# wenbowen123/iros20-6d-pose-tracking

Hardware: NVIDIA H100
Metric: rgbd_pair_frames_per_sec (higher is better)
Workload: dtype bf16x3 (bf16 hi/lo split operands, 3 products/MAC, fp32 accumulate)

## Files before the change

include/se3tn.h:

```cpp
#ifndef SE3TN_H
#define SE3TN_H

#include <stddef.h>
#include <stdint.h>

#ifdef __cplusplus
extern "C" {
#endif

typedef struct se3tn_ctx se3tn_ctx;

enum {
    SE3TN_OK = 0,
    SE3TN_ERR_INVALID = -1,
    SE3TN_ERR_CUDA = -2,
    SE3TN_ERR_NOMEM = -3,
    SE3TN_ERR_STATE = -4,
    SE3TN_ERR_UNSUPPORTED = -5
};

enum {
    SE3TN_PREC_TF32 = 0,
    SE3TN_PREC_FP32 = 1,
    SE3TN_PREC_BF16X3 = 2,
// ... 102 lines not shown

int se3tn_track_render_host(se3tn_ctx* ctx, const uint8_t* frame_rgb, const uint16_t* frame_depth, int H, int W, const double* K,
                            const double* poses, const double* object_width, int render_mode, int render_H, int render_W,
                            const int32_t* weight_ids, int n, double trans_normalizer, double rot_normalizer, int precision,
                            double* poses_out, float* out_trans, float* out_rot, void* stream);


int se3tn_eval_pairs(se3tn_ctx* ctx, const uint8_t* rgbA, const uint16_t* depthA, const uint8_t* rgbB, const uint16_t* depthB,
                     const double* A_in_cam, const double* B_in_cam,
                     const int32_t* weight_ids_host, const int32_t* weight_ids_dev, int n,
                     double trans_normalizer, double rot_normalizer, int precision,
                     float* out_trans, float* out_rot, float* out_sq, double* out_labels, float* out_sums, void* stream);

int se3tn_pair_loss(se3tn_ctx* ctx, const float* trans, const float* rot, const double* trans_label, const double* rot_label, int n,
                    float* out_sums, void* stream);


int se3tn_debug_buffer(se3tn_ctx* ctx, int id, float** ptr, size_t* floats_per_image);

#define SE3TN_PROFILE_SLOTS 22
int se3tn_set_profiling(se3tn_ctx* ctx, int enable);
int se3tn_get_profile(se3tn_ctx* ctx, float* ms);

#define SE3TN_TRACE_WORDS (14 * 256 * 8)
int se3tn_get_trace(se3tn_ctx* ctx, unsigned long long* out);

int se3tn_last_step_was_graph(se3tn_ctx* ctx);
int se3tn_last_launch_count(se3tn_ctx* ctx);

#ifdef __cplusplus
}
#endif
#endif
```

iros20-6d-pose-tracking_b200/_lib.py:

```python
import ctypes as C
import os

_HERE = os.path.dirname(os.path.abspath(__file__))
LIB_PATH = os.path.join(_HERE, 'libse3tn.so')

OK, ERR_INVALID, ERR_CUDA, ERR_NOMEM, ERR_STATE, ERR_UNSUPPORTED = 0, -1, -2, -3, -4, -5
PREC_TF32, PREC_FP32, PREC_BF16X3, PREC_BF16 = 0, 1, 2, 3
RENDER_VISPY, RENDER_PYRENDER = 0, 1
WEIGHT_BLOB_FLOATS = 13528326
PROFILE_SLOTS = 22

_vp, _i, _d, _sz = C.c_void_p, C.c_int, C.c_double, C.c_size_t

SIGNATURES = {
    'se3tn_workspace_bytes': (_sz, [_i]),
    'se3tn_create': (_i, [_i, _i, _vp, C.POINTER(_vp)]),
    'se3tn_destroy': (None, [_vp]),
    'se3tn_last_error': (C.c_char_p, [_vp]),
    'se3tn_load_weights': (_i, [_vp, _i, _vp, _sz]),
    'se3tn_set_stats': (_i, [_vp, _i, _vp, _vp, _i]),
    'se3tn_preprocess': (_i, [_vp, _vp, _vp, _i, _i, _vp, _vp, _vp, _vp, _vp, _vp, _i, _i, _vp, _vp, _vp, _vp, _vp]),
    'se3tn_normalize': (_i, [_vp, _vp, _vp, _vp, _vp, _vp, _vp, _i, _i, _vp, _vp, _vp]),
    'se3tn_compute_bbox': (_i, [_vp, _vp, _vp, _vp, _vp, _vp, _i, _vp]),
    'se3tn_crop_bbox': (_i, [_vp, _vp, _vp, _i, _i, _vp, _i, _i, _i, _vp, _vp, _vp]),
    'se3tn_forward': (_i, [_vp, _i, _vp, _vp, _i, _vp, _vp, _vp, _i, _vp]),
    'se3tn_forward_preprocessed': (_i, [_vp, _i, _i, _i, _vp, _vp, _vp, _i, _vp]),
    'se3tn_pose_update': (_i, [_vp, _vp, _vp, _vp, _d, _d, _vp, _i, _vp]),
    'se3tn_so3_log': (_i, [_vp, _vp, _vp, _d, _d, _vp, _vp, _i, _vp]),
    'se3tn_track_batch': (_i, [_vp, _vp, _vp, _i, _i, _vp, _vp, _vp, _vp, _vp, _vp, _vp, _i, _d, _d, _i, _vp, _vp, _vp, _vp]),
    'se3tn_add_adi': (_i, [_vp, _vp, _i, _vp, _vp, _i, _vp, _vp, _vp]),
    'se3tn_vocap': (_i, [_vp, _vp, _i, C.POINTER(_d), _vp]),
    'se3tn_allgather_poses': (_i, [_vp, _vp, _vp, _vp, _i, _vp]),
    'se3tn_upload_frame_window': (_i, [_vp, _vp, _vp, _i, _i, _i, _i, _i, _i, _vp, _vp, _vp]),
# ... 53 lines not shown
```

iros20-6d-pose-tracking_b200/csrc/conv_common.h:

```cpp
#pragma once
#include <cstdint>
#include <cuda.h>
#include <cuda_runtime.h>

namespace se3tn {

constexpr int kMaxTaps = 9;
constexpr int kBlockM = 128;
constexpr int kChunkBytes = 128;

enum Act : int { ACT_NONE = 0, ACT_RELU = 1, ACT_SELU = 2 };
enum { KIND_S1 = 0, KIND_S2 = 1, KIND_STEM = 2 };

struct Tap {
    int16_t dy, dx;
};

struct ConvGeom {
    int Hin, Win, in_cstride, in_coff;
    int Ho, Wo, stride;
    int cin;
    int cout;
    int groups;
    int num_taps;
// ... 49 lines not shown
    int n_layers;
    int total_units;
    int img_first, n_img;
    int max_batch;
    unsigned* sched;
    const int* img_wid;
    const CUtensorMap* gbmaps;
    const float* const* gbias;
    unsigned long long* trace;
    int ksplit;
    float* partial;
    unsigned* slice_cnt;
};

struct ResidentParams {
    LayerDesc L;
    int img_first, n_img;
    int m_tiles;
    int step_x, step_y, off_x, off_y;
    const int* img_wid;
    const CUtensorMap* gbmaps;
    const float* const* gbias;
    unsigned long long* trace;
};

cudaError_t launch_conv_resident(const ResidentParams& p, int kind, int prec, int num_sms, bool pdl, cudaStream_t stream);
cudaError_t launch_conv_trunk(const TrunkParams& p, int prec, int num_sms, bool pdl, cudaStream_t stream);
constexpr int kSplitMaxImages = 4, kSplitK = 4, kSplitMaxUnits = kSplitMaxImages * 8 * kTrunkMaxLayers;
inline size_t trunk_sched_words(int max_batch) { return 1 + static_cast<size_t>(kTrunkMaxLayers) * max_batch + static_cast<size_t>(kSplitMaxUnits) * 4; }
inline size_t trunk_partial_floats() { return static_cast<size_t>(kSplitMaxUnits) * kSplitK * 128 * 128; }

cudaError_t launch_conv_direct(const ConvGeom& g, const ConvPtrs& p, cudaStream_t stream);

}
```

iros20-6d-pose-tracking_b200/csrc/conv_wgmma.cu:

```cuda
#include "conv_common.h"
#include "ptx.cuh"
#include "storage.cuh"
#include <algorithm>

namespace se3tn {
namespace {

constexpr int kThreads2 = 384;
constexpr int kPoolPitch = 68;
constexpr int kPoolStageBytes = 121 * kPoolPitch * 4;
constexpr int kPoolStageAlloc = (kPoolStageBytes + 1023) & ~1023;
constexpr int kAUnit3 = 19 * 1024;
constexpr int kAUnitStem = 21 * 1024;
constexpr int kWgRowBytes = 64 * kChunkBytes;

template <int KIND> struct KTab;
template <> struct KTab<KIND_S1> {
    static constexpr int NU = 3;
    __host__ __device__ static constexpr int ntaps(int) { return 3; }
    __host__ __device__ static constexpr int wtap(int u, int k) { return k * 3 + u; }
    __host__ __device__ static constexpr int amap(int) { return 0; }
    __host__ __device__ static constexpr int c1(int u) { return u - 1; }
    __host__ __device__ static constexpr int c2(int) { return -1; }
    __host__ __device__ static constexpr int rows(int) { return 11 * 13; }
// ... 13 lines not shown
    __host__ __device__ static constexpr int wtap(int u, int k) { return 2 * k + u; }
    __host__ __device__ static constexpr int amap(int u) { return u; }
    __host__ __device__ static constexpr int c1(int) { return 0; }
    __host__ __device__ static constexpr int c2(int) { return 0; }
    __host__ __device__ static constexpr int rows(int u) { return u == 0 ? 11 * 14 : 11 * 13; }
};
constexpr int kRowShift = 11;

__device__ __forceinline__ float selu_fast(float x) {
    constexpr float kAlpha = 1.6732632423543772f, kScale = 1.0507009873554805f;
    return x > 0.f ? kScale * x : (kScale * kAlpha) * (__expf(x) - 1.f);
}
__device__ __forceinline__ float act_apply(float x, int act) {
    return act == ACT_RELU ? fmaxf(x, 0.f) : (act == ACT_SELU ? selu_fast(x) : x);
}

__device__ __forceinline__ unsigned long long gtimer() { unsigned long long t; asm volatile("mov.u64 %0, %%globaltimer;" : "=l"(t)); return t; }
__device__ __forceinline__ void trace_stamp(unsigned long long* tr, int slot) { if (tr) tr[blockIdx.x * 8 + slot] = gtimer(); }
__device__ __forceinline__ void trace_exit(unsigned long long* tr) {
    if (!tr) return;
    unsigned smid; asm volatile("mov.u32 %0, %%smid;" : "=r"(smid));
    tr[blockIdx.x * 8 + 7] = (gtimer() & ~0xffull) | (smid & 0xff);
}

using ptx::desc_lo;
using ptx::mk_desc;

__device__ __forceinline__ float (&acc_lo32(float (&d)[64]))[32] { return *reinterpret_cast<float (*)[32]>(&d[0]); }

struct Consumer {
    int ct, cg, cw, ew, lane, R, m;
    __device__ __forceinline__ Consumer() {
        ct = static_cast<int>(threadIdx.x) - 128; cg = ct >> 7; ew = ct >> 5; cw = ew & 3; lane = ct & 31; R = lane >> 2; m = lane & 3;
    }
    __device__ __forceinline__ bool leader() const { return (ct & 127) == 0; }
    __device__ __forceinline__ int row(int h) const { return 64 * cg + 16 * cw + R + 8 * h; }
};

template <int KIND, int PREC> struct RCfg {
    static constexpr bool POOL = (KIND == KIND_STEM);
    static constexpr int BN = 64;
    static constexpr int kStack = ((POOL ? stem_input_prec(PREC) : PREC) == SE3TN_PREC_BF16X3) ? 2 : 1;
    static constexpr int kBTile = BN * kStack * kChunkBytes;
    static constexpr int kAUnit = POOL ? kAUnitStem : kAUnit3;
    static constexpr int kAStages = POOL ? (PREC == SE3TN_PREC_TF32 ? 4 : 3) : (PREC == SE3TN_PREC_BF16 ? 6 : 4);
    static constexpr int kPoolBufs = POOL ? (PREC == SE3TN_PREC_TF32 ? 2 : 1) : 0;
    static constexpr int kAcc = BN * kStack / 2;
    static constexpr int kMaxWTiles = POOL ? 7 : ((PREC == SE3TN_PREC_TF32) ? 18 : 9);
    static constexpr int kSmem = kAStages * kAUnit + kMaxWTiles * kBTile + kPoolBufs * kPoolStageAlloc + 1024 + 512;
    static_assert(kSmem <= 232448, "shared memory budget");
};

template <int KIND, int PREC>
__device__ __forceinline__ void resident_mma_unit(float (&acc)[RCfg<KIND, PREC>::kAcc], uint32_t a_unit_lo, const uint8_t* sB,
                                                  int u, int ch, int tiles_per_tap, uint32_t& fresh)
{
    using C = RCfg<KIND, PREC>;
    using KT = KTab<KIND>;
#pragma unroll
    for (int k = 0; k < 4; ++k) {
// ... 2 lines not shown
        uint32_t b_lo;
        if (C::kStack == 2) b_lo = desc_lo(sB + KT::wtap(u, k) * C::kBTile) + ch * 4;
        else                b_lo = desc_lo(sB + (KT::wtap(u, k) * tiles_per_tap + ch) * C::kBTile);
        if constexpr (PREC == SE3TN_PREC_TF32) {
#pragma unroll
            for (int kk = 0; kk < 4; ++kk) ptx::wgmma_tf32_n64(acc, mk_desc(a_lo + 2 * kk), mk_desc(b_lo + 2 * kk), fresh | (kk ? 1u : 0u));
        } else if constexpr (C::POOL) {
#pragma unroll
            for (int kk = 0; kk < 4; ++kk) ptx::wgmma_bf16_n128(acc, mk_desc(a_lo + 2 * kk), mk_desc(b_lo + 2 * kk), fresh | (kk ? 1u : 0u));
        } else if constexpr (C::kStack == 2) {
#pragma unroll
            for (int sl = 0; sl < 2; ++sl) {
                ptx::wgmma_bf16_n128(acc, mk_desc(a_lo + 2 * sl), mk_desc(b_lo + 2 * sl), fresh | (sl ? 1u : 0u));
                ptx::wgmma_bf16_n64(acc_lo32(acc), mk_desc(a_lo + 4 + 2 * sl), mk_desc(b_lo + 2 * sl), 1u);
            }
        } else {
#pragma unroll
            for (int kk = 0; kk < 4; ++kk) ptx::wgmma_bf16_n64(acc, mk_desc(a_lo + 2 * kk), mk_desc(b_lo + 2 * kk), fresh | (kk ? 1u : 0u));
        }
        fresh = 1u;
    }
}

template <int KIND, int PREC>
__global__ void __launch_bounds__(kThreads2, 1)
conv_resident_kernel(const __grid_constant__ ResidentParams p)
{
    using C = RCfg<KIND, PREC>;
    using KT = KTab<KIND>;
    constexpr bool POOL = C::POOL;
    extern __shared__ uint8_t smem_raw[];
    uint8_t* smem = reinterpret_cast<uint8_t*>((reinterpret_cast<uintptr_t>(smem_raw) + 1023) & ~uintptr_t(1023));
    const LayerDesc& L = p.L;
    const int chunks = L.chunks;
    const int tiles_per_tap = (C::kStack == 2) ? 1 : chunks;
    uint8_t* sA = smem;
    uint8_t* sB = sA + C::kAStages * C::kAUnit;
    uint8_t* sP = sB + C::kMaxWTiles * C::kBTile;
    uint64_t* bars = reinterpret_cast<uint64_t*>(sP + C::kPoolBufs * kPoolStageAlloc);
    uint64_t* a_full = bars;
    uint64_t* a_empty = a_full + C::kAStages;
    uint64_t* b_full = a_empty + C::kAStages;
    uint64_t* b_empty = b_full + KT::NU;

    ptx::grid_dep_launch();
    if (threadIdx.x == 0) trace_stamp(p.trace, 0);
    const int warp = threadIdx.x >> 5;
    const int lane = threadIdx.x & 31;
    const int tiles_img = L.tiles_x * L.tiles_y;
    const int w_begin = static_cast<int>(static_cast<long long>(blockIdx.x) * p.m_tiles / gridDim.x);
    const int w_end = static_cast<int>(static_cast<long long>(blockIdx.x + 1) * p.m_tiles / gridDim.x);
    auto img_of = [&](int tile) -> int { return p.img_first + tile / tiles_img; };
    auto wid_of = [&](int tile) -> int { return p.img_wid ? p.img_wid[img_of(tile)] : -1; };

    if (threadIdx.x == 0) {
        for (int s = 0; s < C::kAStages; ++s) { ptx::mbar_init(&a_full[s], 1); ptx::mbar_init(&a_empty[s], 2); }
        for (int u = 0; u < KT::NU; ++u) ptx::mbar_init(&b_full[u], 1);
        ptx::mbar_init(&b_empty[0], 2);
        ptx::fence_barrier_init();
        ptx::fence_proxy_async();
    }
    __syncthreads();
    if (threadIdx.x == 0) trace_stamp(p.trace, 1);

    if (warp == 0) {
        if (lane == 0) {
            ptx::grid_dep_wait();
            int stage = 0; uint32_t phase = 0;
            for (int tile = w_begin; tile < w_end; ++tile) {
                const int n0 = img_of(tile), r = tile % tiles_img;
                const int ty = r / L.tiles_x, tx = r - ty * L.tiles_x;
                const int ox = tx * p.step_x + p.off_x, oy = ty * p.step_y + p.off_y;
                for (int ch = 0; ch < chunks; ++ch) {
#pragma unroll
                    for (int u = 0; u < KT::NU; ++u) {
                        ptx::mbar_wait(&a_empty[stage], phase ^ 1);
                        ptx::mbar_arrive_expect_tx(&a_full[stage], static_cast<uint32_t>(KT::rows(u)) * kChunkBytes);
                        ptx::tma_load_4d(sA + stage * C::kAUnit, &L.amap[KT::amap(u)], &a_full[stage],
                                         ch * 32, ox + KT::c1(u), oy + KT::c2(u), n0);
                        if (++stage == C::kAStages) { stage = 0; phase ^= 1; }
                    }
                }
            }
        }
    } else if (warp == 1) {
        if (lane == 0) {
            int cur = -2; uint32_t gen = 0;
            for (int tile = w_begin; tile < w_end; ++tile) {
                const int wid = wid_of(tile);
                if (wid == cur) continue;
                if (gen) ptx::mbar_wait(&b_empty[0], (gen - 1) & 1);
                const CUtensorMap* bm = wid < 0 ? &L.bmap : p.gbmaps + wid * kLayersPerSet + L.li;
#pragma unroll
                for (int u = 0; u < KT::NU; ++u) {
                    ptx::mbar_arrive_expect_tx(&b_full[u], static_cast<uint32_t>(KT::ntaps(u) * tiles_per_tap) * C::kBTile);
#pragma unroll
                    for (int k = 0; k < KT::ntaps(u); ++k)
                        for (int c = 0; c < tiles_per_tap; ++c) {
                            const int wt = KT::wtap(u, k) * tiles_per_tap + c;
                            ptx::tma_load_2d(sB + wt * C::kBTile, bm, &b_full[u], wt * 32, 0);
                        }
                }
                cur = wid; ++gen;
            }
        }
    } else if (warp >= 4) {
        ptx::grid_dep_wait();
        const Consumer cs;
        const bool stamp = threadIdx.x == 128;
        int astage = 0; uint32_t aphase = 0;
        int w_cur = -2; uint32_t w_gen = 0;
        int it = 0;
        for (int tile = w_begin; tile < w_end; ++tile, ++it) {
            const int wid = wid_of(tile);
            const bool new_w = (wid != w_cur);
            const int n0 = img_of(tile), r = tile % tiles_img;
            const int ty = r / L.tiles_x, tx = r - ty * L.tiles_x;

            using S = Storage<PREC>;
            size_t rpix[2]; bool rvalid[2]; Raw<PREC, 8> rres[2][2];
            if constexpr (!POOL) {
#pragma unroll
                for (int h = 0; h < 2; ++h) {
                    const int rw = cs.row(h);
                    const int py = rw / 11, px = rw - py * 11;
                    const int y = ty * 11 + py, x = tx * 11 + px;
                    rvalid[h] = (rw < 121) && (y < L.Ho) && (x < L.Wo);
                    rpix[h] = (static_cast<size_t>(n0) * L.Ho + y) * L.Wo + x;
#pragma unroll
                    for (int b = 0; b < 2; ++b) {
                        rres[h][b] = Raw<PREC, 8>{};
                        if (L.res && rvalid[h]) {
                            const uint8_t* rp = L.res + S::addr(rpix[h], L.res_c, 32 * b + 8 * cs.m);
#pragma unroll
                            for (int q = 0; q < rres[h][b].kPieces; ++q) rres[h][b].set(q, __ldg(rres[h][b].at(rp, q)));
                        }
                    }
                }
            }

            float acc[C::kAcc];
#pragma unroll
            for (int i = 0; i < C::kAcc; ++i) acc[i] = 0.f;
            uint32_t fresh = 0;
            int pend = -1;
            for (int ch = 0; ch < chunks; ++ch) {
#pragma unroll
                for (int u = 0; u < KT::NU; ++u) {
                    if (new_w && ch == 0) {
                        ptx::mbar_wait(&b_full[u], w_gen & 1);
                        if (it == 0 && u == 0 && stamp) trace_stamp(p.trace, 2);
                    }
                    ptx::mbar_wait(&a_full[astage], aphase);
                    if (it == 0 && ch == 0 && u == 0 && stamp) trace_stamp(p.trace, 3);
                    ptx::wgmma_fence();
                    resident_mma_unit<KIND, PREC>(acc, desc_lo(sA + astage * C::kAUnit + cs.cg * kWgRowBytes), sB, u, ch, tiles_per_tap, fresh);
                    ptx::wgmma_commit();
                    ptx::wgmma_wait<1>();
                    if (pend >= 0 && cs.leader()) ptx::mbar_arrive(&a_empty[pend]);
                    pend = astage;
                    if (++astage == C::kAStages) { astage = 0; aphase ^= 1; }
                }
            }
            ptx::wgmma_wait<0>();
            ptx::wgmma_reg_fence(acc);
            if (cs.leader()) {
                ptx::mbar_arrive(&a_empty[pend]);
                if (tile + 1 < w_end && wid_of(tile + 1) != wid) ptx::mbar_arrive(&b_empty[0]);
            }
            if (new_w) { w_cur = wid; ++w_gen; }
            if (it == 0 && stamp) trace_stamp(p.trace, 5);

            if constexpr (!POOL) {
#pragma unroll
                for (int b = 0; b < 2; ++b) {
                    const int ch0 = 32 * b + 8 * cs.m;
                    const float* bias_base = (p.img_wid ? p.gbias[p.img_wid[n0] * kLayersPerSet + L.li] : L.bias) + ch0;
                    const float4 bA = __ldg(reinterpret_cast<const float4*>(bias_base)), bB = __ldg(reinterpret_cast<const float4*>(bias_base + 4));
                    const float bias8[8] = {bA.x, bA.y, bA.z, bA.w, bB.x, bB.y, bB.z, bB.w};
#pragma unroll
                    for (int h = 0; h < 2; ++h) {
                        if (!rvalid[h]) continue;
                        float v[8];
#pragma unroll
                        for (int jj = 0; jj < 4; ++jj)
#pragma unroll
                            for (int e = 0; e < 2; ++e) {
                                const int ri = 16 * b + 4 * jj + 2 * h + e;
                                float a = acc[ri];
                                if constexpr (C::kStack == 2) a += acc[32 + ri];
                                v[2 * jj + e] = a + bias8[2 * jj + e];
                            }
                        if (L.res) {
                            float r[8];
                            S::decode(rres[h][b], r);
#pragma unroll
                            for (int e = 0; e < 8; ++e) v[e] += r[e];
                        }
#pragma unroll
                        for (int e = 0; e < 8; ++e) v[e] = act_apply(v[e], L.act);
                        S::encode(v).store(L.out + S::addr(rpix[h], L.out_c, L.out_coff + ch0));
                    }
                }
            } else {
                float* stage = reinterpret_cast<float*>(sP + (C::kPoolBufs == 2 ? (it & 1) : 0) * kPoolStageAlloc);
#pragma unroll
                for (int h = 0; h < 2; ++h) {
                    const int rw = cs.row(h);
                    if (rw >= 121) continue;
                    const int cy_l = rw / 11, cx_l = rw - cy_l * 11;
                    const int cy = ty * p.step_y + p.off_y + cy_l, cx = tx * p.step_x + p.off_x + cx_l;
                    const bool cvalid = cy >= 0 && cy < 88 && cx >= 0 && cx < 88;
                    float* srow = stage + rw * kPoolPitch + 2 * cs.m;
                    const float ninf = -3.0e38f;
#pragma unroll
                    for (int j = 0; j < 8; ++j) {
                        float a0 = acc[4 * j + 2 * h], a1 = acc[4 * j + 2 * h + 1];
                        if constexpr (C::kStack == 2) { a0 += acc[32 + 4 * j + 2 * h]; a1 += acc[32 + 4 * j + 2 * h + 1]; }
                        *reinterpret_cast<float2*>(srow + 8 * j) = cvalid ? make_float2(a0, a1) : make_float2(ninf, ninf);
                    }
                }
                asm volatile("bar.sync 1, 256;" ::: "memory");

                const float* bias = p.img_wid ? p.gbias[p.img_wid[n0] * kLayersPerSet + L.li] : L.bias;
                for (int v = cs.ct; v < 400; v += 256) {
                    const int pp = v >> 4, c4 = (v & 15) * 4;
                    const int ppy = pp / 5, ppx = pp - ppy * 5;
                    const int oy = ty * 5 + ppy, ox = tx * 5 + ppx;
                    if (oy >= L.Ho || ox >= L.Wo) continue;
                    float4 mx = make_float4(-3.0e38f, -3.0e38f, -3.0e38f, -3.0e38f);
#pragma unroll
                    for (int dy = 0; dy < 3; ++dy)
#pragma unroll
                        for (int dx = 0; dx < 3; ++dx) {
                            const float4 s4 = *reinterpret_cast<const float4*>(stage + ((2 * ppy + dy) * 11 + 2 * ppx + dx) * kPoolPitch + c4);
                            mx.x = fmaxf(mx.x, s4.x); mx.y = fmaxf(mx.y, s4.y); mx.z = fmaxf(mx.z, s4.z); mx.w = fmaxf(mx.w, s4.w);
                        }
                    const float4 b4 = __ldg(reinterpret_cast<const float4*>(bias + c4));
                    const float v4[4] = {selu_fast(mx.x + b4.x), selu_fast(mx.y + b4.y), selu_fast(mx.z + b4.z), selu_fast(mx.w + b4.w)};
                    S::encode(v4).store(L.out + S::addr((static_cast<size_t>(n0) * L.Ho + oy) * L.Wo + ox, L.out_c, L.out_coff + c4));
                }
                if (C::kPoolBufs == 1) asm volatile("bar.sync 1, 256;" ::: "memory");
            }
        }
        if (stamp) { trace_stamp(p.trace, 4); trace_stamp(p.trace, 6); }
    }

    __syncthreads();
    if (threadIdx.x == 0) trace_exit(p.trace);
}

template <int PREC> struct TCfg {
    static constexpr int BN = 128;
    static constexpr int kAcc = BN / 2;
    static constexpr int kAStages = 3;
    static constexpr int kBStages = 6;
    static constexpr int kBTile = BN * kChunkBytes;
    static constexpr int kEpiPitch = 36;
    static constexpr int kEpiWarpBytes = 16 * kEpiPitch * 4 + 128;
    static constexpr int kEpiBytes = 8 * kEpiWarpBytes;
    static constexpr int kSched = 4;
    static constexpr int kSmem = kAStages * kAUnit3 + kBStages * kBTile + ((kEpiBytes + 1023) & ~1023) + 1024 + 512;
    static_assert(kSmem <= 232448, "shared memory budget");
};
constexpr int kProducerRegs = 40;
constexpr int kConsumerRegs = 232;
constexpr int kTurnBar = 1;
constexpr int kTaps3 = 9;

__device__ __forceinline__ void ring_skip(int& stage, uint32_t& phase, int n, int stages) {
    stage += n;
    phase ^= static_cast<uint32_t>(stage / stages) & 1u;
    stage %= stages;
}

struct UnitCoord { int l, img, tx, ty, n_tile, grp, c0, c1, piece, gidx; };
__device__ __forceinline__ void unit_stamp(const TrunkParams& p, int u, int k) {
    if (p.trace && u < 2048) p.trace[256 * 8 + u * 5 + k] = k == 4 ? (gtimer() & ~0xffull) | (blockIdx.x & 0xff) : gtimer();
}

__device__ __forceinline__ int unit_layer(const TrunkParams& p, int u) {
    int l = 0;
#pragma unroll
    for (int i = 1; i < kTrunkMaxLayers; ++i) if (i < p.n_layers && u >= p.layer[i].unit_base) l = i;
    return l;
}

__device__ __forceinline__ UnitCoord decode_unit(const TrunkParams& p, int u) {
    UnitCoord c;
    c.l = unit_layer(p, u);
    const LayerDesc& L = p.layer[c.l];
    int local = u - L.unit_base;
    c.piece = 0; c.c0 = 0; c.c1 = L.chunks;
    if (p.ksplit > 1) {
        c.piece = local % p.ksplit; local /= p.ksplit;
        c.c0 = c.piece * L.chunks / p.ksplit; c.c1 = (c.piece + 1) * L.chunks / p.ksplit;
    }
// ... 395 lines not shown
    __syncthreads();
    if (threadIdx.x == 0) trace_exit(p.trace);
}

template <typename K>
cudaError_t set_smem(K kernel, size_t smem, size_t* cache) {
    int dev = 0;
    if (cudaGetDevice(&dev) != cudaSuccess || dev < 0 || dev >= 64) dev = 0;
    if (smem > cache[dev]) {
        cudaError_t e = cudaFuncSetAttribute(kernel, cudaFuncAttributeMaxDynamicSharedMemorySize, static_cast<int>(smem));
        if (e != cudaSuccess) return e;
        cache[dev] = smem;
    }
    return cudaSuccess;
}

template <int KIND, int PREC>
cudaError_t launch_resident_t(const ResidentParams& p, int num_sms, bool pdl, cudaStream_t stream) {
    using C = RCfg<KIND, PREC>;
    const int tiles_per_tap = (C::kStack == 2) ? 1 : p.L.chunks;
    if ((KIND == KIND_STEM ? 7 : 9) * tiles_per_tap > C::kMaxWTiles) return cudaErrorInvalidValue;
    if (C::kStack == 2 && KIND == KIND_S1 && p.L.chunks != 2) return cudaErrorInvalidValue;
    if (p.L.cout != 64 || p.L.groups != 1 || p.L.n_tiles != 1 || p.m_tiles <= 0) return cudaErrorInvalidValue;
    static size_t attr[64] = {};
    cudaError_t e = set_smem(conv_resident_kernel<KIND, PREC>, C::kSmem, attr);
    if (e != cudaSuccess) return e;
    cudaLaunchConfig_t cfg = {};
    cfg.gridDim = dim3(std::min(p.m_tiles, num_sms)); cfg.blockDim = dim3(kThreads2); cfg.dynamicSmemBytes = C::kSmem; cfg.stream = stream;
    cudaLaunchAttribute at[1];
    at[0].id = cudaLaunchAttributeProgrammaticStreamSerialization; at[0].val.programmaticStreamSerializationAllowed = 1;
    cfg.attrs = at; cfg.numAttrs = pdl ? 1 : 0;
    return cudaLaunchKernelEx(&cfg, conv_resident_kernel<KIND, PREC>, p);
}

template <int PREC>
cudaError_t launch_trunk_t(const TrunkParams& p, int num_sms, bool pdl, cudaStream_t stream) {
    using C = TCfg<PREC>;
    if (p.n_layers < 1 || p.n_layers > kTrunkMaxLayers || p.total_units <= 0 || !p.sched) return cudaErrorInvalidValue;
    if (p.ksplit < 1 || (p.ksplit > 1 && (!p.partial || !p.slice_cnt || p.ksplit > kSplitK))) return cudaErrorInvalidValue;
    for (int l = 0; l < p.n_layers; ++l) {
        const LayerDesc& L = p.layer[l];
        if ((L.kind != KIND_S1 && L.kind != KIND_S2) || L.cout % C::BN || L.n_tiles != L.cout / C::BN) return cudaErrorInvalidValue;
        if (L.pool_part && (L.tiles_x != 1 || L.tiles_y != 1)) return cudaErrorInvalidValue;
        if (L.dep_layer >= l) return cudaErrorInvalidValue;
        if (L.chunks % p.ksplit) return cudaErrorInvalidValue;
    }
    static size_t attr[64] = {};
    cudaError_t e = set_smem(conv_trunk_kernel<PREC>, C::kSmem, attr);
    if (e != cudaSuccess) return e;
    cudaLaunchConfig_t cfg = {};
    cfg.gridDim = dim3(std::min(p.total_units, num_sms)); cfg.blockDim = dim3(kThreads2); cfg.dynamicSmemBytes = C::kSmem; cfg.stream = stream;
    cudaLaunchAttribute at[1];
    at[0].id = cudaLaunchAttributeProgrammaticStreamSerialization; at[0].val.programmaticStreamSerializationAllowed = 1;
    cfg.attrs = at; cfg.numAttrs = pdl ? 1 : 0;
    return cudaLaunchKernelEx(&cfg, conv_trunk_kernel<PREC>, p);
// ... 32 lines not shown
```

iros20-6d-pose-tracking_b200/csrc/se3tn.cu:

```cuda
#include "../../include/se3tn.h"
#include "conv_common.h"
#include "aux_kernels.h"
#include "metrics.h"
#include "render.h"
#include <dlfcn.h>
#include "depth_fill.h"
#include "storage.cuh"

#include <algorithm>
#include <cmath>
#include <cstdio>
#include <cstdlib>
#include <cstring>
#include <map>
#include <memory>
#include <string>
#include <type_traits>
#include <vector>

using namespace se3tn;

namespace {

enum Buf { B_X0A, B_X0B, B_Y1A, B_Y1B, B_P1A, B_P1B, B_T1, B_T2, B_U, B_CAT, B_F1, B_T4, B_F2, B_H1, B_H2, B_H3, B_COUNT };
// ... 450 lines not shown
            p.w = w.blob.get() + w.w_off[li]; p.bias = w.blob.get() + w.b_off[li];
            { ProfScope ps(c, li, s); CU_TRY(c, launch_conv_direct(g, p, s)); }
            ++c->launches;
            if (li == 0) { ProfScope ps(c, 14, s); CU_TRY(c, launch_maxpool(bufp(B_Y1A), bufp(B_P1A), n, 88, 88, 64, s)); ++c->launches; }
            if (li == 1) { ProfScope ps(c, 15, s); CU_TRY(c, launch_maxpool(bufp(B_Y1B), bufp(B_P1B), n, 88, 88, 64, s)); ++c->launches; }
        }
        { ProfScope ps(c, 16, s); CU_TRY(c, launch_head(bufp(B_H3), fcw, fcw + 6 * 512, out_trans, out_rot, n, 121, s)); }
        ++c->launches;
        if (out_feature) { CU_TRY(c, launch_nhwc_to_nchw(bufp(B_F2), out_feature, n, 22 * 22, 256, precision, s)); ++c->launches; }
        return SE3TN_OK;
    }
    const CUtensorMap* gbmaps = img_wid ? c->d_bmaps[precision].get() : nullptr;
    const float* const* gbias = img_wid ? c->d_bias.get() : nullptr;
    if (c->sched_dirty) { CU_TRY(c, cudaMemsetAsync(c->sched.get(), 0, trunk_sched_words(c->max_batch) * sizeof(unsigned), s)); c->sched_dirty = false; }
    for (int li = 0; li < kFirstTrunkLayer; ++li) {
        ResidentParams rp;
        fill_layer_desc(c, w, li, precision, rp.L);
        rp.img_first = first; rp.n_img = n;
        rp.m_tiles = n * rp.L.tiles_x * rp.L.tiles_y;
        if (kLayers[li].kind == K_STEM) { rp.step_x = rp.step_y = 10; rp.off_x = rp.off_y = -1; }
        else { rp.step_x = rp.step_y = 11; rp.off_x = rp.off_y = 0; }
        rp.img_wid = img_wid; rp.gbmaps = gbmaps; rp.gbias = gbias;
        rp.trace = c->trace ? c->trace.get() + static_cast<size_t>(li) * 256 * 8 : nullptr;
        { ProfScope ps(c, li, s); CU_TRY(c, launch_conv_resident(rp, rp.L.kind, precision, c->num_sms, c->pdl != 0, s)); }
        ++c->launches;
    }
    {
        TrunkParams tp;
        memset(&tp, 0, sizeof tp);
        int ksplit = (n <= kSplitMaxImages) ? kSplitK : 1;
        for (int l = 0; l < 14 - kFirstTrunkLayer; ++l) {
            fill_layer_desc(c, w, kFirstTrunkLayer + l, precision, tp.layer[l]);
            while (tp.layer[l].chunks % ksplit) ksplit /= 2;
        }
        int base = 0, base0 = 0;
        for (int l = 0; l < 14 - kFirstTrunkLayer; ++l) {
            LayerDesc& d = tp.layer[l];
            d.unit_base = base; base += n * d.units_per_image * ksplit;
            d.base_unit0 = base0; base0 += n * d.units_per_image;
            if (l > 0) { d.dep_layer = l - 1; d.dep_target = 4u * static_cast<unsigned>(ksplit) * static_cast<unsigned>(tp.layer[l - 1].units_per_image); }
        }
        if (ksplit > 1 && base0 > kSplitMaxUnits) return fail(c, SE3TN_ERR_STATE, "split-K scratch too small");
        tp.ksplit = ksplit; tp.partial = c->partial.get();
        tp.slice_cnt = c->sched.get() + 1 + static_cast<size_t>(kTrunkMaxLayers) * c->max_batch;
        tp.layer[5].pool_part = c->pool_part.get();
        tp.n_layers = 6; tp.total_units = base;
// ... 888 lines not shown
```

iros20-6d-pose-tracking_b200/engine.py:

```python
import ctypes as C
import math
import numpy as np
import torch

from . import _lib
from .weights import pack_state_dict

PREC = {'tf32': _lib.PREC_TF32, 'fp32': _lib.PREC_FP32, 'bf16x3': _lib.PREC_BF16X3, 'bf16': _lib.PREC_BF16}
IMAGE_SIZE = 176


def _ptr(t):
    return C.c_void_p(t.data_ptr()) if t is not None else C.c_void_p(0)


def _stream(device):
    return C.c_void_p(torch.cuda.current_stream(device).cuda_stream)


class Engine:
    def __init__(self, max_batch=64, device=None):
        if not torch.cuda.is_available():
            raise RuntimeError('se3tn Engine needs a CUDA device (sm_90a); there is no CPU fallback')
        self.lib = _lib.load()
# ... 346 lines not shown
        if not (math.isfinite(max_depth) and max_depth > 0):
            raise ValueError('max_depth must be finite and > 0')
        return (1, max_depth, int(bool(fill_depth.get('extrapolate', False))), 1 if blur_type == 'gaussian' else 0)

    def _set_depth_fill(self, spec):
        _lib.check(self.lib.se3tn_set_depth_fill(self._ctx, int(spec[0]), float(spec[1]), int(spec[2]), int(spec[3])), self._ctx)

    def debug_buffer(self, buf_id, n):
        p = C.c_void_p(); fpi = C.c_size_t()
        _lib.check(self.lib.se3tn_debug_buffer(self._ctx, buf_id, C.byref(p), C.byref(fpi)), self._ctx)
        offb = p.value - self._workspace.data_ptr()
        nbytes = n * fpi.value * 4
        return self._workspace[offb:offb + nbytes].view(torch.float32).view(n, fpi.value)

    def set_profiling(self, enable=True):
        _lib.check(self.lib.se3tn_set_profiling(self._ctx, int(bool(enable))), self._ctx)

    def get_profile(self):
        ms = (C.c_float * _lib.PROFILE_SLOTS)()
        _lib.check(self.lib.se3tn_get_profile(self._ctx, ms), self._ctx)
        return np.array(ms[:], dtype=np.float64)

    def get_trace(self):
        out = np.zeros((14, 256, 8), dtype=np.uint64)
        _lib.check(self.lib.se3tn_get_trace(self._ctx, out.ctypes.data_as(C.c_void_p)), self._ctx)
        return out

    def last_launch_count(self):
        return self.lib.se3tn_last_launch_count(self._ctx)

    def last_step_was_graph(self):
        return bool(self.lib.se3tn_last_step_was_graph(self._ctx))

    def _check_img(self, t):
        if not (t.is_cuda and t.dtype == torch.float32 and t.is_contiguous() and t.dim() == 4 and
                tuple(t.shape[1:]) == (4, IMAGE_SIZE, IMAGE_SIZE)):
            raise ValueError('expected a contiguous float32 CUDA tensor of shape (n,4,176,176), got %s %s' % (t.dtype, tuple(t.shape)))

    def _check_dev(self, name, t, dtype, shape):
        if not (isinstance(t, torch.Tensor) and t.is_cuda and t.device == self.device and t.dtype == dtype and t.is_contiguous()
                and tuple(t.shape) == tuple(shape)):
            raise ValueError('%s must be a contiguous %s CUDA tensor of shape %s on %s' % (name, dtype, tuple(shape), self.device))

    def _check_frame(self, rgb, depth, rgbA, depthA, poses, ow, n):
        ok = (rgb.is_cuda and rgb.dtype == torch.uint8 and rgb.is_contiguous() and rgb.dim() == 3 and rgb.shape[2] == 3 and
              depth.is_cuda and depth.dtype == torch.uint16 and depth.is_contiguous() and depth.shape == rgb.shape[:2] and
              (rgbA is None or (rgbA.is_cuda and rgbA.dtype == torch.uint8 and rgbA.is_contiguous() and tuple(rgbA.shape) == (n, IMAGE_SIZE, IMAGE_SIZE, 3))) and
# ... 33 lines not shown
```

Measured before the change: 27570.

## Ping-pong consumer warpgroups across tiles in resident conv kernel

When a layer has more tiles than SMs, the resident conv kernel now uses a ping-pong schedule. Each consumer warpgroup owns alternate tiles and computes both 64-row halves, and named barriers hand the MMA turn back and forth. This lets one warpgroup's epilogue (bias, residual, activation, pooling) overlap the other's MMAs. Producer and consumer registers are rebalanced with setmaxnreg, and per-tile trace stamps are added for profiling. The trade-offs are higher register pressure from doubled accumulators and extra barrier synchronisation.

```diff
diff --git a/include/se3tn.h b/include/se3tn.h
--- a/include/se3tn.h
+++ b/include/se3tn.h
@@ -148,7 +148,8 @@
 int se3tn_set_profiling(se3tn_ctx* ctx, int enable);
 int se3tn_get_profile(se3tn_ctx* ctx, float* ms);
 
-#define SE3TN_TRACE_WORDS (14 * 256 * 8)
+#define SE3TN_TRACE_TILES 5184
+#define SE3TN_TRACE_WORDS (14 * 256 * 8 + 8 * SE3TN_TRACE_TILES * 4)
 int se3tn_get_trace(se3tn_ctx* ctx, unsigned long long* out);
 
 int se3tn_last_step_was_graph(se3tn_ctx* ctx);
diff --git a/iros20-6d-pose-tracking_b200/_lib.py b/iros20-6d-pose-tracking_b200/_lib.py
--- a/iros20-6d-pose-tracking_b200/_lib.py
+++ b/iros20-6d-pose-tracking_b200/_lib.py
@@ -9,6 +9,7 @@
 RENDER_VISPY, RENDER_PYRENDER = 0, 1
 WEIGHT_BLOB_FLOATS = 13528326
 PROFILE_SLOTS = 22
+TRACE_TILES = 5184
 
 _vp, _i, _d, _sz = C.c_void_p, C.c_int, C.c_double, C.c_size_t
 
diff --git a/iros20-6d-pose-tracking_b200/csrc/conv_common.h b/iros20-6d-pose-tracking_b200/csrc/conv_common.h
--- a/iros20-6d-pose-tracking_b200/csrc/conv_common.h
+++ b/iros20-6d-pose-tracking_b200/csrc/conv_common.h
@@ -95,6 +95,7 @@
     const CUtensorMap* gbmaps;
     const float* const* gbias;
     unsigned long long* trace;
+    unsigned long long* tile_trace;
 };
 
 cudaError_t launch_conv_resident(const ResidentParams& p, int kind, int prec, int num_sms, bool pdl, cudaStream_t stream);
diff --git a/iros20-6d-pose-tracking_b200/csrc/conv_wgmma.cu b/iros20-6d-pose-tracking_b200/csrc/conv_wgmma.cu
--- a/iros20-6d-pose-tracking_b200/csrc/conv_wgmma.cu
+++ b/iros20-6d-pose-tracking_b200/csrc/conv_wgmma.cu
@@ -59,6 +59,9 @@
     unsigned smid; asm volatile("mov.u32 %0, %%smid;" : "=r"(smid));
     tr[blockIdx.x * 8 + 7] = (gtimer() & ~0xffull) | (smid & 0xff);
 }
+__device__ __forceinline__ void tile_stamp(unsigned long long* tt, int tile, int k) {
+    if (tt && tile < SE3TN_TRACE_TILES) tt[tile * 4 + k] = k == 3 ? (gtimer() & ~0xffull) | (blockIdx.x & 0xff) : gtimer();
+}
 
 using ptx::desc_lo;
 using ptx::mk_desc;
@@ -71,8 +74,20 @@
         ct = static_cast<int>(threadIdx.x) - 128; cg = ct >> 7; ew = ct >> 5; cw = ew & 3; lane = ct & 31; R = lane >> 2; m = lane & 3;
     }
     __device__ __forceinline__ bool leader() const { return (ct & 127) == 0; }
-    __device__ __forceinline__ int row(int h) const { return 64 * cg + 16 * cw + R + 8 * h; }
+    __device__ __forceinline__ int row(int half, int h) const { return 64 * half + 16 * cw + R + 8 * h; }
 };
+
+constexpr int kProducerRegs = 40;
+constexpr int kConsumerRegs = 232;
+constexpr int kTurnBar = 1;
+constexpr int kStageBar = 3;
+constexpr int kEpiBar = 5;
+
+__device__ __forceinline__ void ring_skip(int& stage, uint32_t& phase, int n, int stages) {
+    stage += n;
+    phase ^= static_cast<uint32_t>(stage / stages) & 1u;
+    stage %= stages;
+}
 
 template <int KIND, int PREC> struct RCfg {
     static constexpr bool POOL = (KIND == KIND_STEM);
@@ -121,13 +136,15 @@
     }
 }
 
-template <int KIND, int PREC>
+template <int KIND, int PREC, bool PP>
 __global__ void __launch_bounds__(kThreads2, 1)
 conv_resident_kernel(const __grid_constant__ ResidentParams p)
 {
     using C = RCfg<KIND, PREC>;
     using KT = KTab<KIND>;
     constexpr bool POOL = C::POOL;
+    constexpr int NH = PP ? 2 : 1;
+    constexpr bool kShareStage = PP && C::kPoolBufs == 1;
     extern __shared__ uint8_t smem_raw[];
     uint8_t* smem = reinterpret_cast<uint8_t*>((reinterpret_cast<uintptr_t>(smem_raw) + 1023) & ~uintptr_t(1023));
     const LayerDesc& L = p.L;
@@ -153,7 +170,7 @@
     auto wid_of = [&](int tile) -> int { return p.img_wid ? p.img_wid[img_of(tile)] : -1; };
 
     if (threadIdx.x == 0) {
-        for (int s = 0; s < C::kAStages; ++s) { ptx::mbar_init(&a_full[s], 1); ptx::mbar_init(&a_empty[s], 2); }
+        for (int s = 0; s < C::kAStages; ++s) { ptx::mbar_init(&a_full[s], 1); ptx::mbar_init(&a_empty[s], PP ? 1 : 2); }
         for (int u = 0; u < KT::NU; ++u) ptx::mbar_init(&b_full[u], 1);
         ptx::mbar_init(&b_empty[0], 2);
         ptx::fence_barrier_init();
@@ -162,85 +179,117 @@
     __syncthreads();
     if (threadIdx.x == 0) trace_stamp(p.trace, 1);
 
-    if (warp == 0) {
-        if (lane == 0) {
-            ptx::grid_dep_wait();
-            int stage = 0; uint32_t phase = 0;
-            for (int tile = w_begin; tile < w_end; ++tile) {
-                const int n0 = img_of(tile), r = tile % tiles_img;
-                const int ty = r / L.tiles_x, tx = r - ty * L.tiles_x;
-                const int ox = tx * p.step_x + p.off_x, oy = ty * p.step_y + p.off_y;
-                for (int ch = 0; ch < chunks; ++ch) {
+    if (warp < 4) {
+        ptx::setmaxnreg_dec<kProducerRegs>();
+        if (warp == 0) {
+            if (lane == 0) {
+                ptx::grid_dep_wait();
+                int stage = 0; uint32_t phase = 0;
+                for (int tile = w_begin; tile < w_end; ++tile) {
+                    const int n0 = img_of(tile), r = tile % tiles_img;
+                    const int ty = r / L.tiles_x, tx = r - ty * L.tiles_x;
+                    const int ox = tx * p.step_x + p.off_x, oy = ty * p.step_y + p.off_y;
+                    for (int ch = 0; ch < chunks; ++ch) {
+#pragma unroll
+                        for (int u = 0; u < KT::NU; ++u) {
+                            ptx::mbar_wait(&a_empty[stage], phase ^ 1);
+                            ptx::mbar_arrive_expect_tx(&a_full[stage], static_cast<uint32_t>(KT::rows(u)) * kChunkBytes);
+                            ptx::tma_load_4d(sA + stage * C::kAUnit, &L.amap[KT::amap(u)], &a_full[stage],
+                                             ch * 32, ox + KT::c1(u), oy + KT::c2(u), n0);
+                            if (++stage == C::kAStages) { stage = 0; phase ^= 1; }
+                        }
+                    }
+                }
+            }
+        } else if (warp == 1) {
+            if (lane == 0) {
+                int cur = -2; uint32_t gen = 0;
+                for (int tile = w_begin; tile < w_end; ++tile) {
+                    const int wid = wid_of(tile);
+                    if (wid == cur) continue;
+                    if (gen) ptx::mbar_wait(&b_empty[0], (gen - 1) & 1);
+                    const CUtensorMap* bm = wid < 0 ? &L.bmap : p.gbmaps + wid * kLayersPerSet + L.li;
 #pragma unroll
                     for (int u = 0; u < KT::NU; ++u) {
-                        ptx::mbar_wait(&a_empty[stage], phase ^ 1);
-                        ptx::mbar_arrive_expect_tx(&a_full[stage], static_cast<uint32_t>(KT::rows(u)) * kChunkBytes);
-                        ptx::tma_load_4d(sA + stage * C::kAUnit, &L.amap[KT::amap(u)], &a_full[stage],
-                                         ch * 32, ox + KT::c1(u), oy + KT::c2(u), n0);
-                        if (++stage == C::kAStages) { stage = 0; phase ^= 1; }
-                    }
-                }
-            }
-        }
-    } else if (warp == 1) {
-        if (lane == 0) {
-            int cur = -2; uint32_t gen = 0;
-            for (int tile = w_begin; tile < w_end; ++tile) {
-                const int wid = wid_of(tile);
-                if (wid == cur) continue;
-                if (gen) ptx::mbar_wait(&b_empty[0], (gen - 1) & 1);
-                const CUtensorMap* bm = wid < 0 ? &L.bmap : p.gbmaps + wid * kLayersPerSet + L.li;
-#pragma unroll
-                for (int u = 0; u < KT::NU; ++u) {
-                    ptx::mbar_arrive_expect_tx(&b_full[u], static_cast<uint32_t>(KT::ntaps(u) * tiles_per_tap) * C::kBTile);
-#pragma unroll
-                    for (int k = 0; k < KT::ntaps(u); ++k)
-                        for (int c = 0; c < tiles_per_tap; ++c) {
-                            const int wt = KT::wtap(u, k) * tiles_per_tap + c;
-                            ptx::tma_load_2d(sB + wt * C::kBTile, bm, &b_full[u], wt * 32, 0);
-                        }
-                }
-                cur = wid; ++gen;
-            }
-        }
-    } else if (warp >= 4) {
+                        ptx::mbar_arrive_expect_tx(&b_full[u], static_cast<uint32_t>(KT::ntaps(u) * tiles_per_tap) * C::kBTile);
+#pragma unroll
+                        for (int k = 0; k < KT::ntaps(u); ++k)
+                            for (int c = 0; c < tiles_per_tap; ++c) {
+                                const int wt = KT::wtap(u, k) * tiles_per_tap + c;
+                                ptx::tma_load_2d(sB + wt * C::kBTile, bm, &b_full[u], wt * 32, 0);
+                            }
+                    }
+                    cur = wid; ++gen;
+                }
+            }
+        }
+    } else {
+        ptx::setmaxnreg_inc<kConsumerRegs>();
         ptx::grid_dep_wait();
+        using S = Storage<PREC>;
         const Consumer cs;
         const bool stamp = threadIdx.x == 128;
+        const bool tstamp = cs.leader() && (PP || cs.cg == 0);
+        constexpr int kEpiThreads = PP ? 128 : 256;
+        const int et = PP ? (cs.ct & 127) : cs.ct;
+        auto half_of = [&](int hf) { return PP ? hf : cs.cg; };
         int astage = 0; uint32_t aphase = 0;
         int w_cur = -2; uint32_t w_gen = 0;
+        if constexpr (PP) {
+            if (cs.cg == 1) { ptx::bar_arrive(kTurnBar, 256); if constexpr (kShareStage) ptx::bar_arrive(kStageBar, 256); }
+        }
         int it = 0;
         for (int tile = w_begin; tile < w_end; ++tile, ++it) {
             const int wid = wid_of(tile);
             const bool new_w = (wid != w_cur);
+            const bool w_last = tile + 1 < w_end && wid_of(tile + 1) != wid;
+            if (PP && (it & 1) != cs.cg) {
+                ring_skip(astage, aphase, chunks * KT::NU, C::kAStages);
+                if (new_w) {
+#pragma unroll
+                    for (int u = 0; u < KT::NU; ++u) ptx::mbar_wait(&b_full[u], w_gen & 1);
+                    w_cur = wid; ++w_gen;
+                }
+                if (w_last && cs.leader()) ptx::mbar_arrive(&b_empty[0]);
+                continue;
+            }
             const int n0 = img_of(tile), r = tile % tiles_img;
             const int ty = r / L.tiles_x, tx = r - ty * L.tiles_x;
 
-            using S = Storage<PREC>;
-            size_t rpix[2]; bool rvalid[2]; Raw<PREC, 8> rres[2][2];
-            if constexpr (!POOL) {
+            constexpr int kPreRes = (PP && C::kStack == 2) ? 1 : NH;
+            size_t rpix[NH][2]; bool rvalid[NH][2]; Raw<PREC, 8> rres[NH][2][2];
+            auto load_res = [&](int hf) {
 #pragma unroll
                 for (int h = 0; h < 2; ++h) {
-                    const int rw = cs.row(h);
+                    const int rw = cs.row(half_of(hf), h);
                     const int py = rw / 11, px = rw - py * 11;
                     const int y = ty * 11 + py, x = tx * 11 + px;
-                    rvalid[h] = (rw < 121) && (y < L.Ho) && (x < L.Wo);
-                    rpix[h] = (static_cast<size_t>(n0) * L.Ho + y) * L.Wo + x;
+                    rvalid[hf][h] = (rw < 121) && (y < L.Ho) && (x < L.Wo);
+                    rpix[hf][h] = (static_cast<size_t>(n0) * L.Ho + y) * L.Wo + x;
 #pragma unroll
                     for (int b = 0; b < 2; ++b) {
-                        rres[h][b] = Raw<PREC, 8>{};
-                        if (L.res && rvalid[h]) {
-                            const uint8_t* rp = L.res + S::addr(rpix[h], L.res_c, 32 * b + 8 * cs.m);
-#pragma unroll
-                            for (int q = 0; q < rres[h][b].kPieces; ++q) rres[h][b].set(q, __ldg(rres[h][b].at(rp, q)));
+                        rres[hf][h][b] = Raw<PREC, 8>{};
+                        if (L.res && rvalid[hf][h]) {
+                            const uint8_t* rp = L.res + S::addr(rpix[hf][h], L.res_c, 32 * b + 8 * cs.m);
+#pragma unroll
+                            for (int q = 0; q < Raw<PREC, 8>::kPieces; ++q) rres[hf][h][b].set(q, __ldg(Raw<PREC, 8>::at(rp, q)));
                         }
                     }
                 }
-            }
-
-            float acc[C::kAcc];
-#pragma unroll
-            for (int i = 0; i < C::kAcc; ++i) acc[i] = 0.f;
+            };
+            if constexpr (!POOL) {
+#pragma unroll
+                for (int hf = 0; hf < kPreRes; ++hf) load_res(hf);
+            }
+            float4 pb4 = make_float4(0.f, 0.f, 0.f, 0.f);
+            if constexpr (POOL) pb4 = __ldg(reinterpret_cast<const float4*>((p.img_wid ? p.gbias[p.img_wid[n0] * kLayersPerSet + L.li] : L.bias) + (et & 15) * 4));
+
+            float acc[NH][C::kAcc];
+#pragma unroll
+            for (int hf = 0; hf < NH; ++hf)
+#pragma unroll
+                for (int i = 0; i < C::kAcc; ++i) acc[hf][i] = 0.f;
+            if constexpr (PP) ptx::bar_sync(kTurnBar + cs.cg, 256);
             uint32_t fresh = 0;
             int pend = -1;
             for (int ch = 0; ch < chunks; ++ch) {
@@ -251,9 +300,18 @@
                         if (it == 0 && u == 0 && stamp) trace_stamp(p.trace, 2);
                     }
                     ptx::mbar_wait(&a_full[astage], aphase);
-                    if (it == 0 && ch == 0 && u == 0 && stamp) trace_stamp(p.trace, 3);
+                    if (ch == 0 && u == 0) {
+                        if (it == 0 && stamp) trace_stamp(p.trace, 3);
+                        if (tstamp) tile_stamp(p.tile_trace, tile, 0);
+                    }
                     ptx::wgmma_fence();
-                    resident_mma_unit<KIND, PREC>(acc, desc_lo(sA + astage * C::kAUnit + cs.cg * kWgRowBytes), sB, u, ch, tiles_per_tap, fresh);
+                    const uint32_t a_unit_lo = desc_lo(sA + astage * C::kAUnit);
+#pragma unroll
+                    for (int hf = 0; hf < NH; ++hf) {
+                        uint32_t f = fresh;
+                        resident_mma_unit<KIND, PREC>(acc[hf], a_unit_lo + half_of(hf) * (kWgRowBytes >> 4), sB, u, ch, tiles_per_tap, f);
+                    }
+                    fresh = 1u;
                     ptx::wgmma_commit();
                     ptx::wgmma_wait<1>();
                     if (pend >= 0 && cs.leader()) ptx::mbar_arrive(&a_empty[pend]);
@@ -261,68 +319,79 @@
                     if (++astage == C::kAStages) { astage = 0; aphase ^= 1; }
                 }
             }
+            if constexpr (PP) ptx::bar_arrive(kTurnBar + (cs.cg ^ 1), 256);
             ptx::wgmma_wait<0>();
-            ptx::wgmma_reg_fence(acc);
+#pragma unroll
+            for (int hf = 0; hf < NH; ++hf) ptx::wgmma_reg_fence(acc[hf]);
+            if (tstamp) tile_stamp(p.tile_trace, tile, 1);
             if (cs.leader()) {
                 ptx::mbar_arrive(&a_empty[pend]);
-                if (tile + 1 < w_end && wid_of(tile + 1) != wid) ptx::mbar_arrive(&b_empty[0]);
+                if (w_last) ptx::mbar_arrive(&b_empty[0]);
             }
             if (new_w) { w_cur = wid; ++w_gen; }
             if (it == 0 && stamp) trace_stamp(p.trace, 5);
+            if (tstamp) tile_stamp(p.tile_trace, tile, 2);
 
             if constexpr (!POOL) {
 #pragma unroll
-                for (int b = 0; b < 2; ++b) {
-                    const int ch0 = 32 * b + 8 * cs.m;
-                    const float* bias_base = (p.img_wid ? p.gbias[p.img_wid[n0] * kLayersPerSet + L.li] : L.bias) + ch0;
-                    const float4 bA = __ldg(reinterpret_cast<const float4*>(bias_base)), bB = __ldg(reinterpret_cast<const float4*>(bias_base + 4));
-                    const float bias8[8] = {bA.x, bA.y, bA.z, bA.w, bB.x, bB.y, bB.z, bB.w};
-#pragma unroll
-                    for (int h = 0; h < 2; ++h) {
-                        if (!rvalid[h]) continue;
-                        float v[8];
-#pragma unroll
-                        for (int jj = 0; jj < 4; ++jj)
-#pragma unroll
-                            for (int e = 0; e < 2; ++e) {
-                                const int ri = 16 * b + 4 * jj + 2 * h + e;
-                                float a = acc[ri];
-                                if constexpr (C::kStack == 2) a += acc[32 + ri];
-                                v[2 * jj + e] = a + bias8[2 * jj + e];
+                for (int hf = 0; hf < NH; ++hf) {
+                    if (hf >= kPreRes) load_res(hf);
+#pragma unroll
+                    for (int b = 0; b < 2; ++b) {
+                        const int ch0 = 32 * b + 8 * cs.m;
+                        const float* bias_base = (p.img_wid ? p.gbias[p.img_wid[n0] * kLayersPerSet + L.li] : L.bias) + ch0;
+                        const float4 bA = __ldg(reinterpret_cast<const float4*>(bias_base)), bB = __ldg(reinterpret_cast<const float4*>(bias_base + 4));
+                        const float bias8[8] = {bA.x, bA.y, bA.z, bA.w, bB.x, bB.y, bB.z, bB.w};
+#pragma unroll
+                        for (int h = 0; h < 2; ++h) {
+                            if (!rvalid[hf][h]) continue;
+                            float v[8];
+#pragma unroll
+                            for (int jj = 0; jj < 4; ++jj)
+#pragma unroll
+                                for (int e = 0; e < 2; ++e) {
+                                    const int ri = 16 * b + 4 * jj + 2 * h + e;
+                                    float a = acc[hf][ri];
+                                    if constexpr (C::kStack == 2) a += acc[hf][32 + ri];
+                                    v[2 * jj + e] = a + bias8[2 * jj + e];
+                                }
+                            if (L.res) {
+                                float r[8];
+                                S::decode(rres[hf][h][b], r);
+#pragma unroll
+                                for (int e = 0; e < 8; ++e) v[e] += r[e];
                             }
-                        if (L.res) {
-                            float r[8];
-                            S::decode(rres[h][b], r);
-#pragma unroll
-                            for (int e = 0; e < 8; ++e) v[e] += r[e];
+#pragma unroll
+                            for (int e = 0; e < 8; ++e) v[e] = act_apply(v[e], L.act);
+                            S::encode(v).store(L.out + S::addr(rpix[hf][h], L.out_c, L.out_coff + ch0));
                         }
-#pragma unroll
-                        for (int e = 0; e < 8; ++e) v[e] = act_apply(v[e], L.act);
-                        S::encode(v).store(L.out + S::addr(rpix[h], L.out_c, L.out_coff + ch0));
                     }
                 }
             } else {
                 float* stage = reinterpret_cast<float*>(sP + (C::kPoolBufs == 2 ? (it & 1) : 0) * kPoolStageAlloc);
-#pragma unroll
-                for (int h = 0; h < 2; ++h) {
-                    const int rw = cs.row(h);
-                    if (rw >= 121) continue;
-                    const int cy_l = rw / 11, cx_l = rw - cy_l * 11;
-                    const int cy = ty * p.step_y + p.off_y + cy_l, cx = tx * p.step_x + p.off_x + cx_l;
-                    const bool cvalid = cy >= 0 && cy < 88 && cx >= 0 && cx < 88;
-                    float* srow = stage + rw * kPoolPitch + 2 * cs.m;
-                    const float ninf = -3.0e38f;
-#pragma unroll
-                    for (int j = 0; j < 8; ++j) {
-                        float a0 = acc[4 * j + 2 * h], a1 = acc[4 * j + 2 * h + 1];
-                        if constexpr (C::kStack == 2) { a0 += acc[32 + 4 * j + 2 * h]; a1 += acc[32 + 4 * j + 2 * h + 1]; }
-                        *reinterpret_cast<float2*>(srow + 8 * j) = cvalid ? make_float2(a0, a1) : make_float2(ninf, ninf);
-                    }
-                }
-                asm volatile("bar.sync 1, 256;" ::: "memory");
-
-                const float* bias = p.img_wid ? p.gbias[p.img_wid[n0] * kLayersPerSet + L.li] : L.bias;
-                for (int v = cs.ct; v < 400; v += 256) {
+                if constexpr (kShareStage) ptx::bar_sync(kStageBar + cs.cg, 256);
+                else if constexpr (PP) ptx::bar_sync(kEpiBar + cs.cg, 128);
+#pragma unroll
+                for (int hf = 0; hf < NH; ++hf)
+#pragma unroll
+                    for (int h = 0; h < 2; ++h) {
+                        const int rw = cs.row(half_of(hf), h);
+                        if (rw >= 121) continue;
+                        const int cy_l = rw / 11, cx_l = rw - cy_l * 11;
+                        const int cy = ty * p.step_y + p.off_y + cy_l, cx = tx * p.step_x + p.off_x + cx_l;
+                        const bool cvalid = cy >= 0 && cy < 88 && cx >= 0 && cx < 88;
+                        float* srow = stage + rw * kPoolPitch + 2 * cs.m;
+                        const float ninf = -3.0e38f;
+#pragma unroll
+                        for (int j = 0; j < 8; ++j) {
+                            float a0 = acc[hf][4 * j + 2 * h], a1 = acc[hf][4 * j + 2 * h + 1];
+                            if constexpr (C::kStack == 2) { a0 += acc[hf][32 + 4 * j + 2 * h]; a1 += acc[hf][32 + 4 * j + 2 * h + 1]; }
+                            *reinterpret_cast<float2*>(srow + 8 * j) = cvalid ? make_float2(a0, a1) : make_float2(ninf, ninf);
+                        }
+                    }
+                ptx::bar_sync(PP ? kEpiBar + cs.cg : kEpiBar, kEpiThreads);
+
+                for (int v = et; v < 400; v += kEpiThreads) {
                     const int pp = v >> 4, c4 = (v & 15) * 4;
                     const int ppy = pp / 5, ppx = pp - ppy * 5;
                     const int oy = ty * 5 + ppy, ox = tx * 5 + ppx;
@@ -335,12 +404,16 @@
                             const float4 s4 = *reinterpret_cast<const float4*>(stage + ((2 * ppy + dy) * 11 + 2 * ppx + dx) * kPoolPitch + c4);
                             mx.x = fmaxf(mx.x, s4.x); mx.y = fmaxf(mx.y, s4.y); mx.z = fmaxf(mx.z, s4.z); mx.w = fmaxf(mx.w, s4.w);
                         }
-                    const float4 b4 = __ldg(reinterpret_cast<const float4*>(bias + c4));
-                    const float v4[4] = {selu_fast(mx.x + b4.x), selu_fast(mx.y + b4.y), selu_fast(mx.z + b4.z), selu_fast(mx.w + b4.w)};
+                    const float v4[4] = {selu_fast(mx.x + pb4.x), selu_fast(mx.y + pb4.y), selu_fast(mx.z + pb4.z), selu_fast(mx.w + pb4.w)};
                     S::encode(v4).store(L.out + S::addr((static_cast<size_t>(n0) * L.Ho + oy) * L.Wo + ox, L.out_c, L.out_coff + c4));
                 }
-                if (C::kPoolBufs == 1) asm volatile("bar.sync 1, 256;" ::: "memory");
-            }
+                if constexpr (kShareStage) ptx::bar_arrive(kStageBar + (cs.cg ^ 1), 256);
+                else if constexpr (!PP) { if (C::kPoolBufs == 1) ptx::bar_sync(kEpiBar, 256); }
+            }
+            if (tstamp) tile_stamp(p.tile_trace, tile, 3);
+        }
+        if constexpr (PP) {
+            if ((it & 1) == cs.cg) { ptx::bar_sync(kTurnBar + cs.cg, 256); if constexpr (kShareStage) ptx::bar_sync(kStageBar + cs.cg, 256); }
         }
         if (stamp) { trace_stamp(p.trace, 4); trace_stamp(p.trace, 6); }
     }
@@ -362,16 +435,7 @@
     static constexpr int kSmem = kAStages * kAUnit3 + kBStages * kBTile + ((kEpiBytes + 1023) & ~1023) + 1024 + 512;
     static_assert(kSmem <= 232448, "shared memory budget");
 };
-constexpr int kProducerRegs = 40;
-constexpr int kConsumerRegs = 232;
-constexpr int kTurnBar = 1;
 constexpr int kTaps3 = 9;
-
-__device__ __forceinline__ void ring_skip(int& stage, uint32_t& phase, int n, int stages) {
-    stage += n;
-    phase ^= static_cast<uint32_t>(stage / stages) & 1u;
-    stage %= stages;
-}
 
 struct UnitCoord { int l, img, tx, ty, n_tile, grp, c0, c1, piece, gidx; };
 __device__ __forceinline__ void unit_stamp(const TrunkParams& p, int u, int k) {
@@ -813,15 +877,17 @@
     if ((KIND == KIND_STEM ? 7 : 9) * tiles_per_tap > C::kMaxWTiles) return cudaErrorInvalidValue;
     if (C::kStack == 2 && KIND == KIND_S1 && p.L.chunks != 2) return cudaErrorInvalidValue;
     if (p.L.cout != 64 || p.L.groups != 1 || p.L.n_tiles != 1 || p.m_tiles <= 0) return cudaErrorInvalidValue;
-    static size_t attr[64] = {};
-    cudaError_t e = set_smem(conv_resident_kernel<KIND, PREC>, C::kSmem, attr);
+    const bool pp = p.m_tiles > num_sms;
+    void (*kernel)(ResidentParams) = pp ? conv_resident_kernel<KIND, PREC, true> : conv_resident_kernel<KIND, PREC, false>;
+    static size_t attr[2][64] = {};
+    cudaError_t e = set_smem(kernel, C::kSmem, attr[pp]);
     if (e != cudaSuccess) return e;
     cudaLaunchConfig_t cfg = {};
     cfg.gridDim = dim3(std::min(p.m_tiles, num_sms)); cfg.blockDim = dim3(kThreads2); cfg.dynamicSmemBytes = C::kSmem; cfg.stream = stream;
     cudaLaunchAttribute at[1];
     at[0].id = cudaLaunchAttributeProgrammaticStreamSerialization; at[0].val.programmaticStreamSerializationAllowed = 1;
     cfg.attrs = at; cfg.numAttrs = pdl ? 1 : 0;
-    return cudaLaunchKernelEx(&cfg, conv_resident_kernel<KIND, PREC>, p);
+    return cudaLaunchKernelEx(&cfg, kernel, p);
 }
 
 template <int PREC>
diff --git a/iros20-6d-pose-tracking_b200/csrc/se3tn.cu b/iros20-6d-pose-tracking_b200/csrc/se3tn.cu
--- a/iros20-6d-pose-tracking_b200/csrc/se3tn.cu
+++ b/iros20-6d-pose-tracking_b200/csrc/se3tn.cu
@@ -496,6 +496,7 @@
         else { rp.step_x = rp.step_y = 11; rp.off_x = rp.off_y = 0; }
         rp.img_wid = img_wid; rp.gbmaps = gbmaps; rp.gbias = gbias;
         rp.trace = c->trace ? c->trace.get() + static_cast<size_t>(li) * 256 * 8 : nullptr;
+        rp.tile_trace = c->trace ? c->trace.get() + 14 * 256 * 8 + static_cast<size_t>(li) * SE3TN_TRACE_TILES * 4 : nullptr;
         { ProfScope ps(c, li, s); CU_TRY(c, launch_conv_resident(rp, rp.L.kind, precision, c->num_sms, c->pdl != 0, s)); }
         ++c->launches;
     }
diff --git a/iros20-6d-pose-tracking_b200/engine.py b/iros20-6d-pose-tracking_b200/engine.py
--- a/iros20-6d-pose-tracking_b200/engine.py
+++ b/iros20-6d-pose-tracking_b200/engine.py
@@ -392,7 +392,13 @@
         return np.array(ms[:], dtype=np.float64)
 
     def get_trace(self):
-        out = np.zeros((14, 256, 8), dtype=np.uint64)
+        return self._trace_words()[:14 * 256 * 8].reshape(14, 256, 8)
+
+    def get_tile_trace(self):
+        return self._trace_words()[14 * 256 * 8:].reshape(8, _lib.TRACE_TILES, 4)
+
+    def _trace_words(self):
+        out = np.zeros(14 * 256 * 8 + 8 * _lib.TRACE_TILES * 4, dtype=np.uint64)
         _lib.check(self.lib.se3tn_get_trace(self._ctx, out.ctypes.data_as(C.c_void_p)), self._ctx)
         return out
 
```

After: 28520, median of 6. +3.4%, better.
